# EI-CoreBioinformatics/portcullis

Measured on AMD Instinct MI355X. Metric: junc_reads_per_sec, higher is better.
Workload: dtype int32; 1 GPU; BASELINE configs[2]: synthetic 199999998 paired-end 150-bp reads, 25 contigs of GRCh38 lengths (3088286401 bp), 249999 junctions, orientation FR; reads_total=199999998, junctions_total=249999, contigs=25, reads_rank0=199999998, pairs_rank0=66692850

## Files before the change

### portcullis_amd/csrc/pjb_chain.hip.h

```cpp
#pragma once

constexpr unsigned K6_BLOCKS = 128;

static size_t rows_upper_bound(const pjb_ctx *c) {
    size_t n = c->rows_n;
    for (int k = 0; k < c->n_fl; k++)
        if (c->fl[k].queued) n += c->fl[k].lim.junc_limit;
    return n;
}

static void wait_flight(pjb_ctx *c, Flight &f) {
    if (f.queued) (void)hipEventSynchronize(c->sl[f.slot].ev_done);
}

static int rows_table_reserve(pjb_ctx *c, Flight &f, u32 JL) {
    size_t old = rows_upper_bound(c);
    if (old + JL <= c->rows_cap) return PJB_OK;
    for (int k = 0; k < c->n_fl; k++)
        if (c->fl[k].queued && &c->fl[k] != &f) wait_flight(c, c->fl[k]);
    int rc = rows_sync(c);
    if (rc) return rc;
    old = std::min(old, c->rows_cap);
    const size_t ncap = std::max<size_t>((old + JL) * 3 / 2, 1024);
    pjb_junction_row *nd = nullptr;
// ... 473 lines not shown
            else rc = sort_pass<u64>(ch, p == 0 ? S.okey.p : S.key[cur].p, S.key[cur ^ 1].p, vin, vout, shift, bits, ch.d_P, ch.rs_tiles, rs_names);
        }
        if (rc) return rc;
        cur ^= 1;
        shift += bits;
    }
    f.n_pass = ch.n_pass;
    if (ch.run_route) {
        const u32 *order = ch.ro_idx[cur];
        if ((rc = run_scan(c, ro_names[4], RunCountFn{(const u32 *)ro.cnt, order}, RunDestSink{ch.run_dest, order}, (u64)ch.run_cap, ch.ro_total, (const u32 *)ro.n_runs)))
            return rc;
        cur = 1;
        LAUNCH(c, ro_names[5], rs_place, dim3(ch.rs_tiles), dim3(256), (const u32 *)S.jidbam.p, ch.d_P, (const u64 *)ro.key, (const u32 *)ch.run_dest,
               (const u32 *)ro.tile_first, (const u32 *)ro.tile_n, ch.run_cap, ro.tile_bits, (u32 *)S.key[cur].p, (u32 *)S.idx[cur].p);
        f.n_pass = 1;
    }
    ch.cur = cur;
    f.sidx = (const u32 *)S.idx[cur].p;
    f.jid_sorted = f.lim.dense ? (const u32 *)S.key[cur].p : (const u32 *)S.jid.p;
    STAGE_EVENT(2);
    return PJB_OK;
}

static int chain_entropy(Chain &ch) {
    pjb_ctx *c = ch.c;
    CtlSlot &S = ch.S;
    LAUNCH(c, "k5_entropy_sum", k5_entropy_sum, dim3(std::max<u32>(1, (ch.JL + 15) / 16)), dim3(256), (const u32 *)S.seg.p, (const u32 *)S.runfirst.p,
           (const u32 *)S.runstart.p, ch.d_J, (double *)S.entsum.p);
    return PJB_OK;
}

#ifdef PJB_DEBUG_LAUNCH
static void debug_sort_check(Chain &ch) {
    Flight &f = ch.f;
    CtlSlot &S = ch.S;
    const int cur = ch.cur;
    fprintf(stderr, "[k4_pairs] tid %d PL %u JL %u slots_lim %u n_slices_lim %u frag cap %zu fragj cap %zu masks cap %zu rec cap %zu idx cap %zu key cap %zu jkey cap %zu cur %d n_pass %d\n",
            f.tid, ch.PL, ch.JL, ch.slots_lim, ch.n_slices_lim, S.frag.cap, S.fragj.cap, S.masks.cap, S.rec.cap, S.idx[cur].cap, S.key[cur].cap, S.jkey.cap, cur, f.n_pass);
    ContigStats hcs;
    (void)hipDeviceSynchronize();
    (void)hipMemcpy(&hcs, ch.d_cs, sizeof hcs, hipMemcpyDeviceToHost);
    u64 htot = 0;
    (void)hipMemcpy(&htot, S.total.p, 8, hipMemcpyDeviceToHost);
    fprintf(stderr, "[k4_pairs] cs: P %u n_pairs %llu J %u n_junc %u n_slots %u n_slices %u n_cand %u overflow %u R %u total %llu slot %d attempt %d\n", hcs.P,
            (unsigned long long)hcs.n_pairs, hcs.J, hcs.n_junc, hcs.n_slots, hcs.n_slices, hcs.n_cand, hcs.overflow, hcs.R, (unsigned long long)htot, f.slot, f.attempt);
    std::vector<u32> hs(hcs.P), hj(hcs.P), hb(hcs.P);
    (void)hipMemcpy(hs.data(), f.sidx, (size_t)hcs.P * 4, hipMemcpyDeviceToHost);
    (void)hipMemcpy(hj.data(), f.jid_sorted, (size_t)hcs.P * 4, hipMemcpyDeviceToHost);
    (void)hipMemcpy(hb.data(), S.jidbam.p, (size_t)hcs.P * 4, hipMemcpyDeviceToHost);
    std::vector<char> seen(hcs.P, 0);
    size_t bad_idx = 0, dup = 0, bad_order = 0, bad_in = 0, mism = 0;
    long first_bad = -1;
    for (size_t i = 0; i < hcs.P; i++) {
        if (hb[i] >= hcs.J) bad_in++;
        if (hs[i] >= hcs.P) {
            bad_idx++;
            if (first_bad < 0) first_bad = (long)i;
            continue;
        }
        if (seen[hs[i]]) dup++;
        seen[hs[i]] = 1;
        if (hj[i] != hb[hs[i]]) mism++;
        if (i && hj[i] < hj[i - 1]) bad_order++;
    }
    fprintf(stderr, "[k4_pairs] sort check: %zu indices out of range (first at %ld), %zu duplicates, %zu order breaks, %zu key/index mismatches, %zu input ids >= J\n", bad_idx,
            first_bad, dup, bad_order, mism, bad_in);
}
#endif

static int chain_runs_dense(Chain &ch) {
    pjb_ctx *c = ch.c;
    Flight &f = ch.f;
    CtlSlot &S = ch.S;
    const u32 n_slices_lim = ch.n_slices_lim, pair_blocks = ch.pair_blocks;
    int rc;
    u64 *head_mask = (u64 *)S.masks.p, *run_mask = head_mask + n_slices_lim;
    u32 *run_base = (u32 *)(run_mask + n_slices_lim);
    STAGE_EVENT(3);
    STAGE_EVENT(4);
    if (f.forked) HIP_TRY(c, hipStreamWaitEvent(ch.st, S.ev_join, 0));
#ifdef PJB_DEBUG_LAUNCH
    debug_sort_check(ch);
#endif
    LAUNCH(c, "k4_pairs", k4_pairs, dim3(pair_blocks), dim3(256), f.sidx, f.jid_sorted, (const PairRec *)ch.pr.rec, (const u64 *)S.jkey.p, ch.kf, ch.d_P,
           (u32 *)S.frag.p, (int32_t *)S.fragj.p, head_mask, run_mask, (const ContigStats *)ch.d_cs, ch.d_err);
    if ((rc = run_scan(c, "k2_runs", Popc64Fn{(const u64 *)run_mask}, ExclusiveU32Sink{run_base}, (u64)n_slices_lim, (u64 *)S.total.p, &ch.d_cs->n_slices)))
        return rc;
    LAUNCH(c, "k2_expand", k2_expand, dim3((pair_blocks + K2E_PER - 1) / K2E_PER), dim3(256), f.jid_sorted, (const u64 *)head_mask, (const u64 *)run_mask, (const u32 *)run_base,
           (const u64 *)S.total.p, (u32 *)S.seg.p, (u32 *)S.runfirst.p, (u32 *)S.runstart.p, ch.d_cs);
    STAGE_EVENT(5);
    return chain_fork(ch, S.ev_fork2, S.ev_join2, ch.entropy_forked, chain_entropy);
}

static int chain_runs_keys(Chain &ch) {
    pjb_ctx *c = ch.c;
    Flight &f = ch.f;
    CtlSlot &S = ch.S;
    const u32 JL = ch.JL, pair_blocks = ch.pair_blocks;
    int rc;
    const u64 *skey = (const u64 *)S.key[ch.cur].p;
    HeadFn hf{skey, f.sidx, (const PairRec *)ch.pr.rec};
    HeadSink hs{(u32 *)S.jid.p, (u32 *)S.seg.p, (u32 *)S.runfirst.p, (u32 *)S.runstart.p, skey, (u64 *)S.jkey.p, JL};
    if ((rc = run_scan(c, "k2_heads", hf, hs, (u64)ch.PL, (u64 *)S.total.p, ch.d_P))) return rc;
    LAUNCH(c, "k2_close", k2_close, dim3(1), dim3(1), (u64 *)S.total.p, (u32 *)S.seg.p, (u32 *)S.runfirst.p,
           (u32 *)S.runstart.p, ch.d_cs, JL, (const u32 *)ch.d_gen_cnt, ch.gen_cap);
    STAGE_EVENT(3);
    if ((rc = chain_fork(ch, S.ev_fork2, S.ev_join2, ch.entropy_forked, chain_entropy))) return rc;
    LAUNCH(c, "kf_init", kf_init, dim3(std::max<u32>(1, std::min<u32>((JL * F_WORDS + 255) / 256, 4096))), dim3(256), (u32 *)S.acc.p, ch.d_J, (int32_t *)S.ancl.p,
           (int32_t *)S.ancr.p);
    LAUNCH(c, "kf_anchors", kf_anchors, dim3(pair_blocks), dim3(256), f.sidx, (const u32 *)S.jid.p, (const PairRec *)ch.pr.rec, ch.d_P, (u32 *)S.jidbam.p,
           (int32_t *)S.ancl.p, (int32_t *)S.ancr.p);
    if ((rc = chain_k4b(ch))) return rc;
    STAGE_EVENT(4);
    LAUNCH(c, "k4_pairs", k4_pairs, dim3(pair_blocks), dim3(256), f.sidx, f.jid_sorted, (const PairRec *)ch.pr.rec, (const u64 *)S.jkey.p, ch.kf, ch.d_P,
           (u32 *)S.frag.p, (int32_t *)S.fragj.p, (u64 *)nullptr, (u64 *)nullptr, (const ContigStats *)ch.d_cs, ch.d_err);
    STAGE_EVENT(5);
    return PJB_OK;
}

static int chain_rows(Chain &ch) {
    pjb_ctx *c = ch.c;
    Flight &f = ch.f;
    CtlSlot &S = ch.S;
    const hipStream_t st = ch.st;
    const u32 JL = ch.JL;
    LAUNCH(c, "k5_frag_reduce", k5_frag_reduce, dim3((ch.slots_lim + 4 * FRAG_SLOTS_PER_WAVE - 1) / (4 * FRAG_SLOTS_PER_WAVE)), dim3(256),
           (const u32 *)S.frag.p, (const int32_t *)S.fragj.p, ch.d_slots, (u32 *)S.acc.p);
    if (ch.entropy_forked) HIP_TRY(c, hipStreamWaitEvent(st, S.ev_join2, 0));
    LAUNCH(c, "k5_finalize", k5_finalize, dim3(std::max<u32>(1, (JL + 255) / 256)), dim3(256), (const u64 *)S.jkey.p, (const u32 *)S.seg.p,
           (const u32 *)S.runfirst.p, (const u32 *)S.runstart.p, (const u32 *)S.acc.p,
           (const int32_t *)S.ancl.p, (const int32_t *)S.ancr.p, ch.kf, ch.GT, ch.d_J, (const double *)S.entsum.p, (pjb_junction_row *)S.rows.p, ch.d_err,
           ch.d_member_junc);
    STAGE_EVENT(6);
    u64 *mirror_table = nullptr;
    u32 mirror_room = 0;
    if (c->mirror && c->mirror_cap >= PJB_MIRROR_HEADER_BYTES) {
        mirror_table = (u64 *)(c->mirror + PJB_MIRROR_HEADER_BYTES);
        mirror_room = (u32)std::min<size_t>((c->mirror_cap - PJB_MIRROR_HEADER_BYTES) / sizeof(pjb_junction_row), 0xffffffffu);
    }
    const hipStream_t rows_stream = c->side_stream ? c->stream3 : st;
    if (rows_stream != st) {
        HIP_TRY(c, hipEventRecord(S.ev_rows, st));
        HIP_TRY(c, hipStreamWaitEvent(rows_stream, S.ev_rows, 0));
    }
    {
        ChainScope scope{c};
        c->stream = rows_stream;
        LAUNCH(c, "k6_rows_out", k6_rows_out, dim3(K6_BLOCKS), dim3(256), (const u64 *)S.rows.p, (const ContigStats *)ch.d_cs,
               (u64 *)c->rows_table, ch.row_base, ch.mirror_base, (RowCursor *)c->b_cursor.p, mirror_table, mirror_room, ch.d_err, ch.d_gen_cnt, S.pub_dev,
               (const MemberStats *)ch.d_members, ch.d_member_junc, ch.n_members);
    }
    S.at_rest = true;
    HIP_TRY(c, hipEventRecord(S.ev[7], rows_stream));
    HIP_TRY(c, hipEventRecord(S.ev_done, rows_stream));
    f.queued = true;
    return PJB_OK;
}
#undef STAGE_EVENT

static int queue_contig(pjb_ctx *c, Flight &f) {
    Chain ch{c, f, c->sl[f.slot]};
    int rc = chain_plan(ch);
    ChainScope scope{c};
    c->stream = ch.st;
    c->scan_tiles = &ch.S.scan_tiles;
    c->cur_pool = c->cur_slot = f.slot;
    ev_drop(c, f.slot);
    if (rc || (rc = chain_room(ch)) || (rc = chain_front(ch)) || (rc = chain_k1(ch)) || (rc = chain_k2d(ch)) || (rc = chain_sort(ch)) ||
        (rc = f.lim.dense ? chain_runs_dense(ch) : chain_runs_keys(ch)))
        return rc;
    return chain_rows(ch);
}
```

### portcullis_amd/csrc/pjb_kernels.hip.h

```cpp
#pragma once

#include "pjb_device.hip.h"

namespace pjb {

__global__ __launch_bounds__(256) void k0_upper(uint8_t *g, int64_t n, int do_upper, int *has_x) {
    int64_t i = ((int64_t)blockIdx.x * 256 + threadIdx.x) * 16;
    bool x = false;
    for (int64_t j = i; j < n && j < i + 16; j++) {
        uint8_t c = g[j];
        x |= (c == 'X' || (do_upper && c == 'x'));
    }
    if (__ballot(x) && lane_id() == 0) atomicOr(has_x, 1);
    if (!do_upper) return;
    if (i + 16 <= n && ((uintptr_t)(g + i) & 15) == 0) {
        uint4 v = *reinterpret_cast<uint4 *>(g + i);
        u32 *w = reinterpret_cast<u32 *>(&v);
#pragma unroll
        for (int k = 0; k < 4; k++) {
            u32 x = w[k], r = 0;
#pragma unroll
            for (int b = 0; b < 4; b++) {
                u32 c = (x >> (8 * b)) & 0xff;
                if (c >= 'a' && c <= 'z') c -= 32;
// ... 1929 lines not shown
        const u32 q = base + threadIdx.x;
        const bool on = q < n;
        const u32 pc = on ? q : n - 1;
        const u32 rs = cand_rank[pc];
        const u64 k = cand[pc], a = cand_anc[pc];
        bool valid = on && rs < junc_limit;
        u32 id = 0xffffffffu;
        if (valid) {
            int32_t s, e;
            unpack_key(kf, k, s, e);
            id = first_id[rs] + ends_below(ends, rs, (u32)e);
            valid = id < junc_limit;
            if (valid) jkey[id] = k;
        }
        if (valid) {
            const int32_t lo = (int32_t)(u32)a, hi = (int32_t)(u32)(a >> 32);
            if (lo < __hip_atomic_load(&anc_l[id], __ATOMIC_RELAXED, __HIP_MEMORY_SCOPE_AGENT)) atomicMin(&anc_l[id], lo);
            if (hi > __hip_atomic_load(&anc_r[id], __ATOMIC_RELAXED, __HIP_MEMORY_SCOPE_AGENT)) atomicMax(&anc_r[id], hi);
        }
    }
}

enum {
    F_N = 0, F_R1P, F_R1N, F_R2P, F_R2N, F_MS, F_XSP, F_XSN, F_UM, F_BPP, F_PPP, F_REL, F_DIST,
    F_MAXMINANC, F_UP, F_DOWN, F_MAXMMES, F_MAXMINMATCH,
    F_FIRSTMIS,
    F_PAD19,
    F_MISM_LO, F_MISM_HI,
    F_JAD0,
    F_WORDS = 48
};
__device__ __forceinline__ void acc_rest_state(u32 *acc, u64 n_junc) {
    const u64 n = n_junc * F_WORDS, step = (u64)gridDim.x * blockDim.x;
    for (u64 t = (u64)blockIdx.x * blockDim.x + threadIdx.x; t < n; t += step) acc[t] = (t % F_WORDS) == F_FIRSTMIS ? 100000000u : 0u;
}

constexpr int KDA_TILE = 4096;
__device__ __forceinline__ void wave_hist_add(u32 *h, u32 d, bool valid);
constexpr int KDA_PER = 4;
constexpr u32 RUN_W = 2048;
struct RunOut {
    u64 *key;
    u32 *cnt;
    u32 *tile_first;
    u32 *tile_n;
    u32 *n_runs;
    u32 cap;
    u32 window;
    int tile_bits;
};
static_assert(RUN_W == 256 * 8, "kd_assign compacts eight table entries a thread");
__device__ __forceinline__ void runs_close_chain(ContigStats *cs) {
    atomicOr(&cs->overflow, OVF_RUNS);
    cs->P = 0;
    cs->J = 0;
    cs->n_slots = 0;
    cs->n_slices = 0;
}
__global__ __launch_bounds__(256) void kd_assign(const u64 *key, const u32 *np, KeyFmt kf, const u64 *bitmap, const u32 *wrank, const u32 *ends,
                                                 const u32 *first_id, u32 junc_limit, const u64 *total, u32 *jid_bam, u32 *acc, const u64 *jkey,
                                                 const int32_t *anc_l, const int32_t *anc_r, u64 *err, ContigStats *cs_chk, int hist_bits, u32 *hist,
                                                 RunOut ro) {
    __shared__ u32 s_h[4096];
    __shared__ u32 s_run[4];
    __shared__ u32 s_rscan[4];
    const u32 n = *np;
    if (n == 0) {
        if (hist_bits > 0)
            for (u32 d = threadIdx.x; d < (1u << hist_bits); d += 256) hist[(size_t)blockIdx.x * (1u << hist_bits) + d] = 0;
        return;
    }
    {
        const u64 J = *total;
        acc_rest_state(acc, J < (u64)junc_limit ? J : (u64)junc_limit);
    }
    const u32 nb = hist_bits > 0 ? 1u << hist_bits : 0u;
    for (u32 d = threadIdx.x; d < (ro.window ? RUN_W : nb); d += 256) s_h[d] = 0;
    if (threadIdx.x == 0) {
        s_run[0] = 0xffffffffu;
        s_run[1] = 0u;
    }
    if (nb || ro.window) __syncthreads();
    u32 id_lo = 0xffffffffu, id_hi = 0u;
    for (u32 chunk = blockIdx.x * (KDA_TILE / (KDA_PER * 256)); chunk < (blockIdx.x + 1) * (KDA_TILE / (KDA_PER * 256)); chunk++) {
    if (chunk * (KDA_PER * 256) >= n) break;
    u64 kk[KDA_PER];
    u32 pp[KDA_PER];
#pragma unroll
    for (int q = 0; q < KDA_PER; q++) {
        pp[q] = (chunk * KDA_PER + q) * 256 + threadIdx.x;
        kk[q] = key[pp[q] < n ? pp[q] : n - 1];
    }
    bool lead[KDA_PER];
    int32_t ss[KDA_PER], ee[KDA_PER];
    u64 bw[KDA_PER];
    u32 wr[KDA_PER];
#pragma unroll
    for (int q = 0; q < KDA_PER; q++) {
        const u32 plo = (u32)__builtin_amdgcn_update_dpp(0, (int)(u32)kk[q], 0x138, 0xf, 0xf, false);
        const u32 phi = (u32)__builtin_amdgcn_update_dpp(0, (int)(u32)(kk[q] >> 32), 0x138, 0xf, 0xf, false);
        lead[q] = lane_id() == 0 || plo != (u32)kk[q] || phi != (u32)(kk[q] >> 32);
        unpack_key(kf, kk[q], ss[q], ee[q]);
        bw[q] = 0;
        wr[q] = 0;
        if (lead[q]) {
            bw[q] = bitmap[(u32)ss[q] >> 6];
            wr[q] = wrank[(u32)ss[q] >> 6];
        }
    }
    u32 rs_[KDA_PER], fi[KDA_PER], eb[KDA_PER];
#pragma unroll
    for (int q = 0; q < KDA_PER; q++) {
        rs_[q] = wr[q] + (u32)__popcll(bw[q] & ((1ull << (ss[q] & 63)) - 1ull));
        fi[q] = eb[q] = 0;
        if (lead[q]) {
            fi[q] = first_id[rs_[q]];
            eb[q] = ends_below(ends, rs_[q], (u32)ee[q]);
        }
    }
#pragma unroll
    for (int q = 0; q < KDA_PER; q++) {
        const u64 lm = __ballot(lead[q]) & ((2ull << lane_id()) - 1ull);
        const u32 id = (u32)__shfl((int)(fi[q] + eb[q]), 63 - __clzll((long long)lm), 64);
        fi[q] = id;
        eb[q] = 0;
        if (pp[q] < n) jid_bam[pp[q]] = id;
        if (nb) wave_hist_add(s_h, id & (nb - 1u), pp[q] < n);
        if (ro.window) {
            wave_hist_add(s_h, id & (RUN_W - 1u), pp[q] < n);
            if (pp[q] < n) {
                id_lo = id < id_lo ? id : id_lo;
                id_hi = id > id_hi ? id : id_hi;
            }
        }
    }
#ifdef PJB_SELFCHECK
    const u32 p = pp[0];
    if (p < n) {
    const int32_t s = ss[0], e = ee[0];
    const u32 rs = rs_[0], id = fi[0] + eb[0];
    {
        int bad = 0;
        const uint4 *q = reinterpret_cast<const uint4 *>(ends + (size_t)rs * DENSE_ENDS);
        const uint4 a = q[0], b = q[1];
        const u32 ue = (u32)e;
        if (!((bitmap[(u32)s >> 6] >> (s & 63)) & 1ull)) bad = 6;
        else if (!(a.x == ue || a.y == ue || a.z == ue || a.w == ue || b.x == ue || b.y == ue || b.z == ue || b.w == ue)) bad = 7;
        else if (id >= junc_limit || id >= (u32)*total) bad = 1;
        else if (jkey[id] != key[p]) bad = 2;
        else if (anc_l[id] > s || anc_r[id] < e) bad = 3;
        if (bad) {
            set_error(err, 0xfffff000u + (u32)bad, PJB_ERR_HIP);
            cs_chk->P = 0;
        }
    }
    }
#endif
    }
    if (nb) {
        __syncthreads();
        for (u32 d = threadIdx.x; d < nb; d += 256) hist[(size_t)blockIdx.x * nb + d] = s_h[d];
    }
    if (ro.window) {
        id_lo = wave_total<DppMin>(id_lo);
        id_hi = wave_total<DppMax>(id_hi);
        if (lane_id() == 0) {
            atomicMin(&s_run[0], id_lo);
            atomicMax(&s_run[1], id_hi);
        }
        __syncthreads();
        const u32 lo = s_run[0], hi = s_run[1];
        if (lo > hi) {
            if (threadIdx.x == 0) ro.tile_n[blockIdx.x] = 0;
            return;
        }
        if (hi - lo >= ro.window) {
            if (threadIdx.x == 0) {
                ro.tile_n[blockIdx.x] = 0;
                runs_close_chain(cs_chk);
            }
            return;
        }
        const u32 span = hi - lo + 1u;
        u32 c[8], nz = 0;
#pragma unroll
        for (int k = 0; k < 8; k++) {
            const u32 o = threadIdx.x * 8u + (u32)k;
            c[k] = o < span ? s_h[(lo + o) & (RUN_W - 1u)] : 0u;
            nz += c[k] != 0u;
        }
        u32 tot;
        u32 at = block_escan_256<u32>(nz, s_rscan, &tot);
        if (threadIdx.x == 0) {
            u32 b = atomicAdd(ro.n_runs, tot);
            if (b > ro.cap || tot > ro.cap - b) {
                atomicSub(ro.n_runs, tot);
                b = 0xffffffffu;
                runs_close_chain(cs_chk);
            }
            s_run[2] = b;
            ro.tile_first[blockIdx.x] = b == 0xffffffffu ? 0u : b;
            ro.tile_n[blockIdx.x] = b == 0xffffffffu ? 0u : tot;
        }
        __syncthreads();
        const u32 first = s_run[2];
        if (first == 0xffffffffu) return;
        at += first;
#pragma unroll
        for (int k = 0; k < 8; k++)
            if (c[k]) {
                ro.key[at] = ((u64)(lo + threadIdx.x * 8u + (u32)k) << ro.tile_bits) | (u64)blockIdx.x;
                ro.cnt[at] = c[k];
                at++;
            }
    }
}

constexpr int RS_ITEMS = 16;
constexpr int RS_TILE = 256 * RS_ITEMS;
constexpr int RS_MAX_BITS = 12;
constexpr int RS_MAX_BINS = 1 << RS_MAX_BITS;
static_assert(KDA_TILE == RS_TILE && RS_MAX_BINS <= 4096, "kd_assign counts the sort's first digit tile by tile");

__device__ __forceinline__ void wave_hist_add(u32 *h, u32 d, bool valid) {
    u64 rem = __ballot(valid);
    const int lane = lane_id();
#pragma unroll
    for (int it = 0; it < 2; it++) {
        if (rem == 0) return;
        const int first = __ffsll((long long)rem) - 1;
        const u32 d0 = __shfl(d, first, 64);
        const u64 m = __ballot(valid && d == d0) & rem;
        if (lane == first) atomicAdd(&h[d0], (u32)__popcll(m));
        rem &= ~m;
    }
    if ((rem >> lane) & 1ull) atomicAdd(&h[d], 1u);
}

template <typename K>
__global__ __launch_bounds__(256) void rs_hist(const K *keys, const u32 *np, int shift, int bits, u32 *hist, u32 n_tiles) {
// ... 608 lines not shown
        if (threadIdx.x == 255) s_first[2 * GEN_SHARDS] = total;
        __syncthreads();
    }
    static_assert(GEN_SHARDS == 256, "two sub-lists per thread of the block");
    const u32 n_items = s_first[2 * GEN_SHARDS];
    for (u32 item0 = blockIdx.x * 256; item0 < n_items; item0 += gridDim.x * 256) {
    const u32 item = item0 + threadIdx.x;
    if (item >= n_items) continue;
    u32 sub = 0;
#pragma unroll
    for (u32 step = GEN_SHARDS; step > 0; step >>= 1)
        if (sub + step < 2 * GEN_SHARDS && s_first[sub + step] <= item) sub += step;
    const bool check_only = sub >= GEN_SHARDS;
    const u64 entry = list[(size_t)sub * cap + (item - s_first[sub])];
    const u32 p0 = (u32)(entry >> 32);
    const u32 slot = check_only && pack_nn ? (u32)entry & 0x0fffffffu : (u32)entry;
    if (check_only) {
        const u32 code = pack_nn ? (u32)entry >> 28 : 15u;
        const u32 nN = code < 15u ? code : (reinterpret_cast<const uint4 *>(rec + p0)[1].w >> 16) + 1u;
        bool ok = true;
        int32_t prev_istart = 0, is, ie;
        unpack_key(kf, key[p0], is, ie);
        for (u32 k = 0; k < nN; k++) {
            const u32 j = jid_bam[p0 + k];
            int32_t nis = 0, nie = 0;
            if (k + 1 < nN) unpack_key(kf, key[p0 + k + 1], nis, nie);
            if (k > 0 && prev_istart >= anc_l[j]) ok = false;
            if (k + 1 < nN && nie + 1 <= anc_r[j]) ok = false;
            prev_istart = is;
            is = nis;
            ie = nie;
        }
        if (ok) continue;
    }
    const int bi = s_bt.find(batches, n_batches, slot / (u32)K1_TILE);
    const DevBatch &b = batches[bi];
    const u32 r = spl_idx[slot];
    const uint4 sr = spl_rec[slot];
    const u32 g = gload(&b.base) + r;
    const u32 c0 = sr.x;
    u32 nc = sr.w & 0x7fffu;
    if (nc == 0x7fffu) nc = gload(b.cig_off + r + 1) - c0;
    OpsView cig;
    cig.g = b.cigar + c0;
    cig.lds = &s_ops[0][threadIdx.x];
    {
        u32 w[OPS_LDS];
        fetch_ops8(as_global(b.cigar), c0, s_bt.cig_words(b, bi), w);
#pragma unroll
        for (int k = 0; k < OPS_LDS; k++) s_ops[k][threadIdx.x] = (u32)k < nc ? w[k] : 0u;
    }
    const uint4 rb = reinterpret_cast<const uint4 *>(rec + p0)[1];
    const int32_t vpos = (int32_t)rb.x, aend = (int32_t)rb.y;
    const Member M = member_of(G, vpos);
    const int32_t pos = vpos - M.voff;
    int32_t lq = (int32_t)(sr.w >> 16);
    if (lq == 0xffff) lq = gload(b.l_qseq + r);
    const u32 so0 = sr.z;
    if (lq > 1 && !(sr.w & 0x8000u)) {
        set_error(err, g, PJB_ERR_NO_SEQ);
        continue;
    }
    const uint8_t *seq = b.seq4 + (size_t)so0 * 4;
    const int32_t q_limit = (int32_t)min(s_bt.seq_words(b, bi) - 1u - so0, 0x7fffffffu);
    u32 k = 0;
    int32_t qsum = 0;
    for (u32 i = 0; i < nc; i++) {
        const u32 op = cig[i], ty = op & 15u;
        if (ty == OP_N) {
            const u32 p = p0 + k;
            const u32 j = jid_bam[p];
            int32_t istart, iend;
            unpack_key(kf, key[p], istart, iend);
            const u64 res = pair_stats_generic(cig, nc, pos, aend - vpos + 1, seq, lq, M.d, M.len, genome_has_x != 0, use_codes ? M.codes : (const u32 *)nullptr,
                                               anc_l[j] - M.voff, istart - M.voff, iend - M.voff, anc_r[j] - M.voff, g, err, i, qsum, q_limit);
            *reinterpret_cast<u64 *>(rec + p) = res;
            k++;
        }
        if (op_consumes_query(ty) && ty != OP_S) qsum += (int32_t)(op >> 4);
    }
    }
}

__global__ __launch_bounds__(256) void k4_pairs(const u32 *sidx, const u32 *jid_of, const PairRec *rec, const u64 *jkey, KeyFmt kf, const u32 *np,
                                                 u32 *frag, int32_t *frag_j, u64 *head_mask, u64 *run_mask, const ContigStats *cs_chk, u64 *err_chk) {
    const u32 n = *np;
    if (blockIdx.x * 256u >= n) return;
    const u32 i = blockIdx.x * 256 + threadIdx.x;
    const bool valid = i < n;
    const int lane = lane_id();
    const u32 ic = valid ? i : n - 1;
    const u32 p = sidx[ic];
    const u32 jv = jid_of[ic];
#ifdef PJB_SELFCHECK
    {
        const u32 Jc = cs_chk->J;
        const u32 jb = ic ? jid_of[ic - 1] : jv;
        int bad = 0;
        if (p >= n) bad = 1;
        else if (jv >= Jc) bad = 2;
        else if (jv != jb && jv != jb + 1) bad = 3;
        else if (ic == 0 && jv != 0) bad = 4;
        else if (ic == n - 1 && jv != Jc - 1) bad = 5;
        else if (jv + (ic >> 6) + 1 >= cs_chk->n_slots) bad = 6;
        else if ((ic >> 6) >= cs_chk->n_slices) bad = 7;
        else if (cs_chk->n_slots != Jc + (n + 63) / 64) bad = 8;
        if (__ballot(bad != 0)) {
            if (bad) set_error(err_chk, 0xffffe000u + (u32)bad, PJB_ERR_HIP);
            return;
        }
    }
#endif
    const PairRec Rc = rec_load(rec + p);
    const u64 jk = jkey[jv];
    u32 jprev_v = __shfl_up(jv, 1, 64);
    int32_t pos_prev = __shfl_up(Rc.pos, 1, 64), aend_prev = __shfl_up(Rc.aend, 1, 64);
    if (lane == 0 && valid && i > 0) {
        jprev_v = jid_of[i - 1];
        const uint4 q = reinterpret_cast<const uint4 *>(rec + sidx[i - 1])[1];
        pos_prev = (int32_t)q.x;
        aend_prev = (int32_t)q.y;
    }
    u32 j = 0xffffffffu;
    u32 cnt[4] = {0, 0, 0, 0}, jadp[5] = {0, 0, 0, 0, 0}, mx[5] = {0, 0, 0, 0, 0};
    u32 first_mis = 100000000u;
    u64 mism64 = 0;
    if (valid) {
        j = jv;
        int32_t istart, iend;
        unpack_key(kf, jk, istart, iend);
        const u64 rs = Rc.aux;
        const u32 minMatch = (u32)(rs & 0xfffffu), mmes = (u32)((rs >> 20) & 0xfffffu), nbMis = (u32)(rs >> 40);
        const u32 meta = Rc.meta;
        const u32 cat = meta & META_CAT_MASK;
        const u32 xs = (meta >> META_XS_SHIFT) & 3u;
        const bool dist_head = i == 0 || jprev_v != j || pos_prev != Rc.pos || aend_prev != Rc.aend;
        cnt[0] = 1u | ((u32)(cat == 0) << 8) | ((u32)(cat == 1) << 16) | ((u32)(cat == 2) << 24);
        cnt[1] = (u32)(cat == 3) | ((u32)((meta & META_MULTI) != 0) << 8) | ((u32)(xs == 1) << 16) | ((u32)(xs == 2) << 24);
        cnt[2] = (u32)((meta & META_UM) != 0) | ((u32)((meta & META_BPP) != 0) << 8) | ((u32)((meta & META_PPP) != 0) << 16) |
                 ((u32)((meta & META_REL) != 0) << 24);
        cnt[3] = (u32)dist_head;
#pragma unroll
        for (int w = 0; w < 5; w++)
            jadp[w] = (u32)((u32)(4 * w) < minMatch) | ((u32)((u32)(4 * w + 1) < minMatch) << 8) |
                      ((u32)((u32)(4 * w + 2) < minMatch) << 16) | ((u32)((u32)(4 * w + 3) < minMatch) << 24);
        const int32_t la = istart - Rc.lstart, ra = Rc.rend - iend;
        mx[0] = (u32)(la < ra ? la : ra);
        mx[1] = Rc.updown & 0xffffu;
        mx[2] = Rc.updown >> 16;
        mx[3] = mmes;
        mx[4] = minMatch;
        first_mis = minMatch > 0 ? minMatch : 100000000u;
        mism64 = nbMis;
        if (lane == 0 && i > 0 && jprev_v != j) frag_j[j + (i >> 6) - 1] = -1;
        if (i == n - 1) frag_j[j + (i >> 6) + 1] = -1;
    }
    if (head_mask) {
        const bool hj = valid && (i == 0 || jprev_v != j);
        const bool hr = valid && (hj || pos_prev != Rc.pos);
        const u64 mj = __ballot(hj), mr = __ballot(hr);
        if (lane == 0 && i < n) {
            head_mask[i >> 6] = mj;
            run_mask[i >> 6] = mr;
        }
    }
    auto store_fragment = [&](u32 hi_word) {
        const u32 slot = j + (i >> 6);
        u32 vals[F_WORDS];
#pragma unroll
        for (int k = 0; k < F_WORDS; k++) vals[k] = 0;
#pragma unroll
        for (int k = 0; k < 13; k++) vals[F_N + k] = (cnt[k >> 2] >> (8 * (k & 3))) & 0xffu;
        vals[F_MAXMINANC] = mx[0];
        vals[F_UP] = mx[1];
        vals[F_DOWN] = mx[2];
        vals[F_MAXMMES] = mx[3];
        vals[F_MAXMINMATCH] = mx[4];
        vals[F_FIRSTMIS] = first_mis;
        vals[F_MISM_LO] = (u32)mism64;
        vals[F_MISM_HI] = hi_word;
#pragma unroll
        for (int k = 0; k < 20; k++) vals[F_JAD0 + k] = (jadp[k >> 2] >> (8 * (k & 3))) & 0xffu;
        uint4 *dst = reinterpret_cast<uint4 *>(frag + (size_t)slot * F_WORDS);
#pragma unroll
        for (int k = 0; k < F_WORDS / 4; k++) dst[k] = make_uint4(vals[4 * k], vals[4 * k + 1], vals[4 * k + 2], vals[4 * k + 3]);
        frag_j[slot] = (int32_t)j;
    };
    const u32 j0 = (u32)__builtin_amdgcn_readfirstlane((int)j);
    if (__ballot(valid && j != j0) == 0) {
#pragma unroll
        for (int w = 0; w < 4; w++) cnt[w] = wave_total<DppAdd>(cnt[w]);
#pragma unroll
        for (int w = 0; w < 5; w++) jadp[w] = wave_total<DppAdd>(jadp[w]);
#pragma unroll
        for (int w = 0; w < 5; w++) mx[w] = wave_total<DppMax>(mx[w]);
        first_mis = wave_total<DppMin>(first_mis);
        mism64 = (u64)wave_total<DppAdd>((u32)mism64);
        if (valid && lane == 0) store_fragment(0u);
        return;
    }
    u32 take = 0;
#pragma unroll
    for (int sft = 0; sft < 6; sft++) {
        const int o = 1 << sft;
        const u32 kk = __shfl_down(j, o, 64);
        if (lane + o < 64 && kk == j) take |= 1u << sft;
    }
    auto red_add = [&](u32 v) {
#pragma unroll
        for (int sft = 0; sft < 6; sft++) {
            const u32 t = __shfl_down(v, 1 << sft, 64);
            if ((take >> sft) & 1u) v += t;
        }
        return v;
    };
    auto red_max = [&](u32 v) {
#pragma unroll
        for (int sft = 0; sft < 6; sft++) {
            const u32 t = __shfl_down(v, 1 << sft, 64);
            if (((take >> sft) & 1u) && t > v) v = t;
        }
        return v;
    };
#pragma unroll
    for (int w = 0; w < 4; w++) cnt[w] = red_add(cnt[w]);
#pragma unroll
    for (int w = 0; w < 5; w++) jadp[w] = red_add(jadp[w]);
#pragma unroll
    for (int w = 0; w < 5; w++) mx[w] = red_max(mx[w]);
#pragma unroll
    for (int sft = 0; sft < 6; sft++) {
        const u32 t = __shfl_down(first_mis, 1 << sft, 64);
        const u64 t64 = __shfl_down(mism64, 1 << sft, 64);
        if ((take >> sft) & 1u) {
            first_mis = t < first_mis ? t : first_mis;
            mism64 += t64;
        }
    }
    const u32 jprev = __shfl_up(j, 1, 64);
    if (valid && (lane == 0 || jprev != j)) store_fragment((u32)(mism64 >> 32));
}

__device__ __forceinline__ u32 frag_combine(int k, u32 a, u32 b) {
    if (k >= F_MAXMINANC && k <= F_MAXMINMATCH) return a > b ? a : b;
    if (k == F_FIRSTMIS) return a < b ? a : b;
    return a + b;
}
constexpr int FRAG_SLOTS_PER_WAVE = 16;
__global__ __launch_bounds__(256) void k5_frag_reduce(const u32 *frag, const int32_t *frag_j, const u32 *n_slots_p, u32 *acc) {
    const u32 n_slots = *n_slots_p;
    const u32 wave = (blockIdx.x * 256 + threadIdx.x) >> 6;
    const int k = lane_id();
    const u32 s0 = wave * FRAG_SLOTS_PER_WAVE;
    if (s0 >= n_slots) return;
    const int32_t myj = (k < FRAG_SLOTS_PER_WAVE && s0 + k < n_slots) ? frag_j[s0 + k] : -1;
    int32_t cur = -1;
    u32 v = 0, carry_lo = 0;
    auto flush = [&](int32_t j) {
        if (j < 0 || k >= F_JAD0 + 20) return;
        u32 *dst = acc + (size_t)j * F_WORDS + k;
        if (k == F_MISM_LO) return;
        if (k == F_MISM_HI) {
            atomicAdd(reinterpret_cast<u64 *>(dst - 1), ((u64)v << 32) | carry_lo);
        } else if (k >= F_MAXMINANC && k <= F_MAXMINMATCH) atomicMax(dst, v);
        else if (k == F_FIRSTMIS) atomicMin(dst, v);
        else if (v) atomicAdd(dst, v);
    };
    u32 row[FRAG_SLOTS_PER_WAVE];
#pragma unroll
    for (int q = 0; q < FRAG_SLOTS_PER_WAVE; q++) {
        const int32_t jq = __shfl(myj, q, 64);
        row[q] = (jq >= 0 && k < F_WORDS) ? frag[(size_t)(s0 + (u32)q) * F_WORDS + k] : 0u;
    }
#pragma unroll
    for (int q = 0; q < FRAG_SLOTS_PER_WAVE; q++) {
        const int32_t j = __shfl(myj, q, 64);
        if (j >= 0) {
            const u32 w = row[q];
            const u32 wlo = __shfl(w, F_MISM_LO, 64);
            if (j != cur) {
                flush(cur);
                cur = j;
                v = w;
                carry_lo = wlo;
            } else if (k == F_MISM_HI) {
                const u64 sum = (((u64)v << 32) | carry_lo) + (((u64)w << 32) | wlo);
                v = (u32)(sum >> 32);
                carry_lo = (u32)sum;
            } else {
                v = frag_combine(k, v, w);
            }
        }
    }
    flush(cur);
}


__global__ __launch_bounds__(256) void k5_entropy_sum(const u32 *seg_off, const u32 *run_first, const u32 *run_start, const u32 *n_junc_p,
                                                       double *ent_sum) {
    const int lane = lane_id(), sl = lane & 15;
    const u32 j = ((blockIdx.x * 4 + (threadIdx.x >> 6)) << 2) + (u32)(lane >> 4);
    const bool valid = j < *n_junc_p;
    const u32 rf = valid ? run_first[j] : 0u, rl = valid ? run_first[j + 1] : 0u;
    const u32 n = valid ? seg_off[j + 1] - seg_off[j] : 0u;
    double sum = 0.0;
    for (u32 r0 = rf; __any(r0 < rl); r0 += 16) {
        const u32 r = r0 + (u32)sl;
        double t = 0.0;
        if (r < rl) {
            u32 c = run_start[r + 1] - run_start[r];
            if (rl - rf > 1) {
                if (r == rf) c += 1;
                else if (r == rl - 1) c -= 1;
            }
            if (c != 0 && n > 1) {
                const double pI = (double)c / (double)n;
                t = __dmul_rn(pI, log2(pI));
            }
        }
        const u32 cnt = r0 < rl ? (rl - r0 < 16u ? rl - r0 : 16u) : 0u;
#pragma unroll
        for (u32 k = 0; k < 16; k++) {
            const double v = __shfl(t, (int)k, 16);
// ... 238 lines not shown
```

Baseline: 30.03 billion reads/s.

## Process multiple slices per wave in k4_pairs and software-pipeline dense-assign chunks

k4_pairs now handles K4_PER consecutive 64-element slices per wave. When all of them share one junction, it folds their counters into a single fragment using widened 16-bit lanes and marks the other fragment slots empty with -1. Previous-element context for later slices comes from readlane instead of a global reload, and the launch grid shrinks to match. Separately, the dense-assign kernel's chunk loop is restructured into staged lambdas so that key loads and bitmap lookups for later chunks are issued before the current chunk finishes, hiding memory latency at the cost of more registers.

```diff
diff --git a/portcullis_amd/csrc/pjb_chain.hip.h b/portcullis_amd/csrc/pjb_chain.hip.h
--- a/portcullis_amd/csrc/pjb_chain.hip.h
+++ b/portcullis_amd/csrc/pjb_chain.hip.h
@@ -579,7 +579,7 @@
 #ifdef PJB_DEBUG_LAUNCH
     debug_sort_check(ch);
 #endif
-    LAUNCH(c, "k4_pairs", k4_pairs, dim3(pair_blocks), dim3(256), f.sidx, f.jid_sorted, (const PairRec *)ch.pr.rec, (const u64 *)S.jkey.p, ch.kf, ch.d_P,
+    LAUNCH(c, "k4_pairs", k4_pairs, dim3((pair_blocks + K4_PER - 1) / K4_PER), dim3(256), f.sidx, f.jid_sorted, (const PairRec *)ch.pr.rec, (const u64 *)S.jkey.p, ch.kf, ch.d_P,
            (u32 *)S.frag.p, (int32_t *)S.fragj.p, head_mask, run_mask, (const ContigStats *)ch.d_cs, ch.d_err);
     if ((rc = run_scan(c, "k2_runs", Popc64Fn{(const u64 *)run_mask}, ExclusiveU32Sink{run_base}, (u64)n_slices_lim, (u64 *)S.total.p, &ch.d_cs->n_slices)))
         return rc;
@@ -609,7 +609,7 @@
            (int32_t *)S.ancl.p, (int32_t *)S.ancr.p);
     if ((rc = chain_k4b(ch))) return rc;
     STAGE_EVENT(4);
-    LAUNCH(c, "k4_pairs", k4_pairs, dim3(pair_blocks), dim3(256), f.sidx, f.jid_sorted, (const PairRec *)ch.pr.rec, (const u64 *)S.jkey.p, ch.kf, ch.d_P,
+    LAUNCH(c, "k4_pairs", k4_pairs, dim3((pair_blocks + K4_PER - 1) / K4_PER), dim3(256), f.sidx, f.jid_sorted, (const PairRec *)ch.pr.rec, (const u64 *)S.jkey.p, ch.kf, ch.d_P,
            (u32 *)S.frag.p, (int32_t *)S.fragj.p, (u64 *)nullptr, (u64 *)nullptr, (const ContigStats *)ch.d_cs, ch.d_err);
     STAGE_EVENT(5);
     return PJB_OK;
diff --git a/portcullis_amd/csrc/pjb_kernels.hip.h b/portcullis_amd/csrc/pjb_kernels.hip.h
--- a/portcullis_amd/csrc/pjb_kernels.hip.h
+++ b/portcullis_amd/csrc/pjb_kernels.hip.h
@@ -2035,80 +2035,103 @@
     }
     if (nb || ro.window) __syncthreads();
     u32 id_lo = 0xffffffffu, id_hi = 0u;
-    for (u32 chunk = blockIdx.x * (KDA_TILE / (KDA_PER * 256)); chunk < (blockIdx.x + 1) * (KDA_TILE / (KDA_PER * 256)); chunk++) {
-    if (chunk * (KDA_PER * 256) >= n) break;
-    u64 kk[KDA_PER];
-    u32 pp[KDA_PER];
-#pragma unroll
-    for (int q = 0; q < KDA_PER; q++) {
-        pp[q] = (chunk * KDA_PER + q) * 256 + threadIdx.x;
-        kk[q] = key[pp[q] < n ? pp[q] : n - 1];
-    }
-    bool lead[KDA_PER];
-    int32_t ss[KDA_PER], ee[KDA_PER];
-    u64 bw[KDA_PER];
-    u32 wr[KDA_PER];
-#pragma unroll
-    for (int q = 0; q < KDA_PER; q++) {
-        const u32 plo = (u32)__builtin_amdgcn_update_dpp(0, (int)(u32)kk[q], 0x138, 0xf, 0xf, false);
-        const u32 phi = (u32)__builtin_amdgcn_update_dpp(0, (int)(u32)(kk[q] >> 32), 0x138, 0xf, 0xf, false);
-        lead[q] = lane_id() == 0 || plo != (u32)kk[q] || phi != (u32)(kk[q] >> 32);
-        unpack_key(kf, kk[q], ss[q], ee[q]);
-        bw[q] = 0;
-        wr[q] = 0;
-        if (lead[q]) {
-            bw[q] = bitmap[(u32)ss[q] >> 6];
-            wr[q] = wrank[(u32)ss[q] >> 6];
-        }
-    }
-    u32 rs_[KDA_PER], fi[KDA_PER], eb[KDA_PER];
-#pragma unroll
-    for (int q = 0; q < KDA_PER; q++) {
-        rs_[q] = wr[q] + (u32)__popcll(bw[q] & ((1ull << (ss[q] & 63)) - 1ull));
-        fi[q] = eb[q] = 0;
-        if (lead[q]) {
-            fi[q] = first_id[rs_[q]];
-            eb[q] = ends_below(ends, rs_[q], (u32)ee[q]);
-        }
-    }
-#pragma unroll
-    for (int q = 0; q < KDA_PER; q++) {
-        const u64 lm = __ballot(lead[q]) & ((2ull << lane_id()) - 1ull);
-        const u32 id = (u32)__shfl((int)(fi[q] + eb[q]), 63 - __clzll((long long)lm), 64);
-        fi[q] = id;
-        eb[q] = 0;
-        if (pp[q] < n) jid_bam[pp[q]] = id;
-        if (nb) wave_hist_add(s_h, id & (nb - 1u), pp[q] < n);
-        if (ro.window) {
-            wave_hist_add(s_h, id & (RUN_W - 1u), pp[q] < n);
-            if (pp[q] < n) {
-                id_lo = id < id_lo ? id : id_lo;
-                id_hi = id > id_hi ? id : id_hi;
-            }
-        }
-    }
+    constexpr int KDA_CHUNKS = KDA_TILE / (KDA_PER * 256);
+    u64 kk[KDA_CHUNKS][KDA_PER];
+    u32 pp[KDA_CHUNKS][KDA_PER];
+    bool lead[KDA_CHUNKS][KDA_PER];
+    int32_t ss[KDA_CHUNKS][KDA_PER], ee[KDA_CHUNKS][KDA_PER];
+    u64 bw[KDA_CHUNKS][KDA_PER];
+    u32 wr[KDA_CHUNKS][KDA_PER];
+    u32 rs_[KDA_CHUNKS][KDA_PER], fi[KDA_CHUNKS][KDA_PER], eb[KDA_CHUNKS][KDA_PER];
+    const auto live = [&](int c) __attribute__((always_inline)) {
+        return c < KDA_CHUNKS && (u64)(blockIdx.x * (u32)KDA_CHUNKS + (u32)c) * (u64)(KDA_PER * 256) < (u64)n;
+    };
+    const auto ask_keys = [&](int c) __attribute__((always_inline)) {
+        if (!live(c)) return;
+#pragma unroll
+        for (int q = 0; q < KDA_PER; q++) {
+            pp[c][q] = ((blockIdx.x * (u32)KDA_CHUNKS + (u32)c) * KDA_PER + q) * 256 + threadIdx.x;
+            kk[c][q] = key[pp[c][q] < n ? pp[c][q] : n - 1];
+        }
+    };
+    const auto ask_words = [&](int c) __attribute__((always_inline)) {
+        if (!live(c)) return;
+#pragma unroll
+        for (int q = 0; q < KDA_PER; q++) {
+            const u32 plo = (u32)__builtin_amdgcn_update_dpp(0, (int)(u32)kk[c][q], 0x138, 0xf, 0xf, false);
+            const u32 phi = (u32)__builtin_amdgcn_update_dpp(0, (int)(u32)(kk[c][q] >> 32), 0x138, 0xf, 0xf, false);
+            lead[c][q] = lane_id() == 0 || plo != (u32)kk[c][q] || phi != (u32)(kk[c][q] >> 32);
+            unpack_key(kf, kk[c][q], ss[c][q], ee[c][q]);
+            bw[c][q] = 0;
+            wr[c][q] = 0;
+            if (lead[c][q]) {
+                bw[c][q] = bitmap[(u32)ss[c][q] >> 6];
+                wr[c][q] = wrank[(u32)ss[c][q] >> 6];
+            }
+        }
+    };
+    const auto ask_slots = [&](int c) __attribute__((always_inline)) {
+        if (!live(c)) return;
+#pragma unroll
+        for (int q = 0; q < KDA_PER; q++) {
+            rs_[c][q] = wr[c][q] + (u32)__popcll(bw[c][q] & ((1ull << (ss[c][q] & 63)) - 1ull));
+            fi[c][q] = eb[c][q] = 0;
+            if (lead[c][q]) {
+                fi[c][q] = first_id[rs_[c][q]];
+                eb[c][q] = ends_below(ends, rs_[c][q], (u32)ee[c][q]);
+            }
+        }
+    };
+    const auto finish = [&](int c) __attribute__((always_inline)) {
+        if (!live(c)) return;
+#pragma unroll
+        for (int q = 0; q < KDA_PER; q++) {
+            const u64 lm = __ballot(lead[c][q]) & ((2ull << lane_id()) - 1ull);
+            const u32 id = (u32)__shfl((int)(fi[c][q] + eb[c][q]), 63 - __clzll((long long)lm), 64);
+            fi[c][q] = id;
+            eb[c][q] = 0;
+            if (pp[c][q] < n) jid_bam[pp[c][q]] = id;
+            if (nb) wave_hist_add(s_h, id & (nb - 1u), pp[c][q] < n);
+            if (ro.window) {
+                wave_hist_add(s_h, id & (RUN_W - 1u), pp[c][q] < n);
+                if (pp[c][q] < n) {
+                    id_lo = id < id_lo ? id : id_lo;
+                    id_hi = id > id_hi ? id : id_hi;
+                }
+            }
+        }
 #ifdef PJB_SELFCHECK
-    const u32 p = pp[0];
-    if (p < n) {
-    const int32_t s = ss[0], e = ee[0];
-    const u32 rs = rs_[0], id = fi[0] + eb[0];
-    {
-        int bad = 0;
-        const uint4 *q = reinterpret_cast<const uint4 *>(ends + (size_t)rs * DENSE_ENDS);
-        const uint4 a = q[0], b = q[1];
-        const u32 ue = (u32)e;
-        if (!((bitmap[(u32)s >> 6] >> (s & 63)) & 1ull)) bad = 6;
-        else if (!(a.x == ue || a.y == ue || a.z == ue || a.w == ue || b.x == ue || b.y == ue || b.z == ue || b.w == ue)) bad = 7;
-        else if (id >= junc_limit || id >= (u32)*total) bad = 1;
-        else if (jkey[id] != key[p]) bad = 2;
-        else if (anc_l[id] > s || anc_r[id] < e) bad = 3;
-        if (bad) {
-            set_error(err, 0xfffff000u + (u32)bad, PJB_ERR_HIP);
-            cs_chk->P = 0;
-        }
-    }
-    }
+        const u32 p = pp[c][0];
+        if (p < n) {
+        const int32_t s = ss[c][0], e = ee[c][0];
+        const u32 rs = rs_[c][0], id = fi[c][0] + eb[c][0];
+        {
+            int bad = 0;
+            const uint4 *q = reinterpret_cast<const uint4 *>(ends + (size_t)rs * DENSE_ENDS);
+            const uint4 a = q[0], b = q[1];
+            const u32 ue = (u32)e;
+            if (!((bitmap[(u32)s >> 6] >> (s & 63)) & 1ull)) bad = 6;
+            else if (!(a.x == ue || a.y == ue || a.z == ue || a.w == ue || b.x == ue || b.y == ue || b.z == ue || b.w == ue)) bad = 7;
+            else if (id >= junc_limit || id >= (u32)*total) bad = 1;
+            else if (jkey[id] != key[p]) bad = 2;
+            else if (anc_l[id] > s || anc_r[id] < e) bad = 3;
+            if (bad) {
+                set_error(err, 0xfffff000u + (u32)bad, PJB_ERR_HIP);
+                cs_chk->P = 0;
+            }
+        }
+        }
 #endif
+    };
+    ask_keys(0);
+    ask_words(0);
+    ask_keys(1);
+#pragma unroll
+    for (int c = 0; c < KDA_CHUNKS; c++) {
+        ask_slots(c);
+        ask_words(c + 1);
+        ask_keys(c + 2);
+        finish(c);
     }
     if (nb) {
         __syncthreads();
@@ -2883,59 +2906,131 @@
     }
 }
 
+constexpr int K4_PER = 2;
+static_assert(K4_PER >= 1 && K4_PER * 64 < 65536 && K4_PER < 256, "the folded sums travel in 16-bit lanes, a lane's own in 8-bit lanes");
 __global__ __launch_bounds__(256) void k4_pairs(const u32 *sidx, const u32 *jid_of, const PairRec *rec, const u64 *jkey, KeyFmt kf, const u32 *np,
                                                  u32 *frag, int32_t *frag_j, u64 *head_mask, u64 *run_mask, const ContigStats *cs_chk, u64 *err_chk) {
     const u32 n = *np;
-    if (blockIdx.x * 256u >= n) return;
-    const u32 i = blockIdx.x * 256 + threadIdx.x;
-    const bool valid = i < n;
     const int lane = lane_id();
-    const u32 ic = valid ? i : n - 1;
-    const u32 p = sidx[ic];
-    const u32 jv = jid_of[ic];
+    const u32 slice0 = (u32)__builtin_amdgcn_readfirstlane((int)((blockIdx.x * 4u + (threadIdx.x >> 6)) * (u32)K4_PER));
+    if ((u64)slice0 * 64u >= n) return;
+    u32 ii[K4_PER], pp[K4_PER], jv[K4_PER];
+#pragma unroll
+    for (int s = 0; s < K4_PER; s++) {
+        ii[s] = (slice0 + (u32)s) * 64u + (u32)lane;
+        const u32 ic = ii[s] < n ? ii[s] : n - 1;
+        pp[s] = sidx[ic];
+        jv[s] = jid_of[ic];
+    }
+    const bool fetch_before = slice0 > 0;
+    u32 p_before = 0, j_before = 0;
+    if (fetch_before) {
+        p_before = sidx[slice0 * 64u - 1u];
+        j_before = jid_of[slice0 * 64u - 1u];
+    }
 #ifdef PJB_SELFCHECK
     {
         const u32 Jc = cs_chk->J;
-        const u32 jb = ic ? jid_of[ic - 1] : jv;
         int bad = 0;
-        if (p >= n) bad = 1;
-        else if (jv >= Jc) bad = 2;
-        else if (jv != jb && jv != jb + 1) bad = 3;
-        else if (ic == 0 && jv != 0) bad = 4;
-        else if (ic == n - 1 && jv != Jc - 1) bad = 5;
-        else if (jv + (ic >> 6) + 1 >= cs_chk->n_slots) bad = 6;
-        else if ((ic >> 6) >= cs_chk->n_slices) bad = 7;
-        else if (cs_chk->n_slots != Jc + (n + 63) / 64) bad = 8;
+#pragma unroll
+        for (int s = 0; s < K4_PER; s++) {
+            const u32 ic = ii[s] < n ? ii[s] : n - 1;
+            const u32 p = pp[s], jvs = jv[s];
+            const u32 jb = ic ? jid_of[ic - 1] : jvs;
+            if (bad) continue;
+            if (p >= n) bad = 1;
+            else if (jvs >= Jc) bad = 2;
+            else if (jvs != jb && jvs != jb + 1) bad = 3;
+            else if (ic == 0 && jvs != 0) bad = 4;
+            else if (ic == n - 1 && jvs != Jc - 1) bad = 5;
+            else if (jvs + (ic >> 6) + 1 >= cs_chk->n_slots) bad = 6;
+            else if ((ic >> 6) >= cs_chk->n_slices) bad = 7;
+            else if (cs_chk->n_slots != Jc + (n + 63) / 64) bad = 8;
+        }
         if (__ballot(bad != 0)) {
             if (bad) set_error(err_chk, 0xffffe000u + (u32)bad, PJB_ERR_HIP);
             return;
         }
     }
 #endif
-    const PairRec Rc = rec_load(rec + p);
-    const u64 jk = jkey[jv];
-    u32 jprev_v = __shfl_up(jv, 1, 64);
-    int32_t pos_prev = __shfl_up(Rc.pos, 1, 64), aend_prev = __shfl_up(Rc.aend, 1, 64);
-    if (lane == 0 && valid && i > 0) {
-        jprev_v = jid_of[i - 1];
-        const uint4 q = reinterpret_cast<const uint4 *>(rec + sidx[i - 1])[1];
-        pos_prev = (int32_t)q.x;
-        aend_prev = (int32_t)q.y;
+    PairRec Rc[K4_PER];
+    u64 jk[K4_PER];
+#pragma unroll
+    for (int s = 0; s < K4_PER; s++) {
+        Rc[s] = rec_load(rec + pp[s]);
+        jk[s] = jkey[jv[s]];
+    }
+    int32_t pos_before = 0, aend_before = 0;
+    if (fetch_before) {
+        const uint4 q = reinterpret_cast<const uint4 *>(rec + p_before)[1];
+        pos_before = (int32_t)q.x;
+        aend_before = (int32_t)q.y;
+    }
+    auto store_fragment = [&](u32 slot, u32 jj, auto sum_of, auto jad_of, const u32(&mxv)[5], u32 fm, u32 mis_lo, u32 mis_hi) {
+        u32 vals[F_WORDS];
+#pragma unroll
+        for (int k = 0; k < F_WORDS; k++) vals[k] = 0;
+#pragma unroll
+        for (int k = 0; k < 13; k++) vals[F_N + k] = sum_of(k);
+        vals[F_MAXMINANC] = mxv[0];
+        vals[F_UP] = mxv[1];
+        vals[F_DOWN] = mxv[2];
+        vals[F_MAXMMES] = mxv[3];
+        vals[F_MAXMINMATCH] = mxv[4];
+        vals[F_FIRSTMIS] = fm;
+        vals[F_MISM_LO] = mis_lo;
+        vals[F_MISM_HI] = mis_hi;
+#pragma unroll
+        for (int k = 0; k < 20; k++) vals[F_JAD0 + k] = jad_of(k);
+        uint4 *dst = reinterpret_cast<uint4 *>(frag + (size_t)slot * F_WORDS);
+#pragma unroll
+        for (int k = 0; k < F_WORDS / 4; k++) dst[k] = make_uint4(vals[4 * k], vals[4 * k + 1], vals[4 * k + 2], vals[4 * k + 3]);
+        frag_j[slot] = (int32_t)jj;
+    };
+    const u32 jw = (u32)__builtin_amdgcn_readfirstlane((int)jv[0]);
+    bool other = false;
+#pragma unroll
+    for (int s = 0; s < K4_PER; s++) other = other || (ii[s] < n && jv[s] != jw);
+    const bool fold = __ballot(other) == 0;
+    u32 fcnt[4] = {0, 0, 0, 0}, fjad[5] = {0, 0, 0, 0, 0}, fmx[5] = {0, 0, 0, 0, 0};
+    u32 ffirst = 100000000u, fmis = 0;
+#pragma unroll
+    for (int s = 0; s < K4_PER; s++) {
+    if ((u64)(slice0 + (u32)s) * 64u < n) {
+    const u32 i = ii[s];
+    const bool valid = i < n;
+    const PairRec &R = Rc[s];
+    u32 jprev_v = __shfl_up(jv[s], 1, 64);
+    int32_t pos_prev = __shfl_up(R.pos, 1, 64), aend_prev = __shfl_up(R.aend, 1, 64);
+    if (s == 0) {
+        if (fetch_before && lane == 0) {
+            jprev_v = j_before;
+            pos_prev = pos_before;
+            aend_prev = aend_before;
+        }
+    } else {
+        const u32 jl = (u32)__builtin_amdgcn_readlane((int)jv[s > 0 ? s - 1 : 0], 63);
+        const int32_t pl = __builtin_amdgcn_readlane(Rc[s > 0 ? s - 1 : 0].pos, 63), al = __builtin_amdgcn_readlane(Rc[s > 0 ? s - 1 : 0].aend, 63);
+        if (lane == 0) {
+            jprev_v = jl;
+            pos_prev = pl;
+            aend_prev = al;
+        }
     }
     u32 j = 0xffffffffu;
     u32 cnt[4] = {0, 0, 0, 0}, jadp[5] = {0, 0, 0, 0, 0}, mx[5] = {0, 0, 0, 0, 0};
     u32 first_mis = 100000000u;
     u64 mism64 = 0;
     if (valid) {
-        j = jv;
+        j = jv[s];
         int32_t istart, iend;
-        unpack_key(kf, jk, istart, iend);
-        const u64 rs = Rc.aux;
+        unpack_key(kf, jk[s], istart, iend);
+        const u64 rs = R.aux;
         const u32 minMatch = (u32)(rs & 0xfffffu), mmes = (u32)((rs >> 20) & 0xfffffu), nbMis = (u32)(rs >> 40);
-        const u32 meta = Rc.meta;
+        const u32 meta = R.meta;
         const u32 cat = meta & META_CAT_MASK;
         const u32 xs = (meta >> META_XS_SHIFT) & 3u;
-        const bool dist_head = i == 0 || jprev_v != j || pos_prev != Rc.pos || aend_prev != Rc.aend;
+        const bool dist_head = i == 0 || jprev_v != j || pos_prev != R.pos || aend_prev != R.aend;
         cnt[0] = 1u | ((u32)(cat == 0) << 8) | ((u32)(cat == 1) << 16) | ((u32)(cat == 2) << 24);
         cnt[1] = (u32)(cat == 3) | ((u32)((meta & META_MULTI) != 0) << 8) | ((u32)(xs == 1) << 16) | ((u32)(xs == 2) << 24);
         cnt[2] = (u32)((meta & META_UM) != 0) | ((u32)((meta & META_BPP) != 0) << 8) | ((u32)((meta & META_PPP) != 0) << 16) |
@@ -2945,10 +3040,10 @@
         for (int w = 0; w < 5; w++)
             jadp[w] = (u32)((u32)(4 * w) < minMatch) | ((u32)((u32)(4 * w + 1) < minMatch) << 8) |
                       ((u32)((u32)(4 * w + 2) < minMatch) << 16) | ((u32)((u32)(4 * w + 3) < minMatch) << 24);
-        const int32_t la = istart - Rc.lstart, ra = Rc.rend - iend;
+        const int32_t la = istart - R.lstart, ra = R.rend - iend;
         mx[0] = (u32)(la < ra ? la : ra);
-        mx[1] = Rc.updown & 0xffffu;
-        mx[2] = Rc.updown >> 16;
+        mx[1] = R.updown & 0xffffu;
+        mx[2] = R.updown >> 16;
         mx[3] = mmes;
         mx[4] = minMatch;
         first_mis = minMatch > 0 ? minMatch : 100000000u;
@@ -2958,37 +3053,27 @@
     }
     if (head_mask) {
         const bool hj = valid && (i == 0 || jprev_v != j);
-        const bool hr = valid && (hj || pos_prev != Rc.pos);
+        const bool hr = valid && (hj || pos_prev != R.pos);
         const u64 mj = __ballot(hj), mr = __ballot(hr);
-        if (lane == 0 && i < n) {
+        if (lane == 0) {
             head_mask[i >> 6] = mj;
             run_mask[i >> 6] = mr;
         }
     }
-    auto store_fragment = [&](u32 hi_word) {
-        const u32 slot = j + (i >> 6);
-        u32 vals[F_WORDS];
-#pragma unroll
-        for (int k = 0; k < F_WORDS; k++) vals[k] = 0;
-#pragma unroll
-        for (int k = 0; k < 13; k++) vals[F_N + k] = (cnt[k >> 2] >> (8 * (k & 3))) & 0xffu;
-        vals[F_MAXMINANC] = mx[0];
-        vals[F_UP] = mx[1];
-        vals[F_DOWN] = mx[2];
-        vals[F_MAXMMES] = mx[3];
-        vals[F_MAXMINMATCH] = mx[4];
-        vals[F_FIRSTMIS] = first_mis;
-        vals[F_MISM_LO] = (u32)mism64;
-        vals[F_MISM_HI] = hi_word;
-#pragma unroll
-        for (int k = 0; k < 20; k++) vals[F_JAD0 + k] = (jadp[k >> 2] >> (8 * (k & 3))) & 0xffu;
-        uint4 *dst = reinterpret_cast<uint4 *>(frag + (size_t)slot * F_WORDS);
-#pragma unroll
-        for (int k = 0; k < F_WORDS / 4; k++) dst[k] = make_uint4(vals[4 * k], vals[4 * k + 1], vals[4 * k + 2], vals[4 * k + 3]);
-        frag_j[slot] = (int32_t)j;
-    };
-    const u32 j0 = (u32)__builtin_amdgcn_readfirstlane((int)j);
-    if (__ballot(valid && j != j0) == 0) {
+    const auto sum8 = [&](int k) { return (cnt[k >> 2] >> (8 * (k & 3))) & 0xffu; };
+    const auto jad8 = [&](int k) { return (jadp[k >> 2] >> (8 * (k & 3))) & 0xffu; };
+    const u32 js = (u32)__builtin_amdgcn_readfirstlane((int)j);
+    if (fold) {
+#pragma unroll
+        for (int w = 0; w < 4; w++) fcnt[w] += cnt[w];
+#pragma unroll
+        for (int w = 0; w < 5; w++) fjad[w] += jadp[w];
+#pragma unroll
+        for (int w = 0; w < 5; w++) fmx[w] = mx[w] > fmx[w] ? mx[w] : fmx[w];
+        ffirst = first_mis < ffirst ? first_mis : ffirst;
+        fmis += (u32)mism64;
+        if (s > 0 && lane == 0) frag_j[jw + slice0 + (u32)s] = -1;
+    } else if (__ballot(valid && j != js) == 0) {
 #pragma unroll
         for (int w = 0; w < 4; w++) cnt[w] = wave_total<DppAdd>(cnt[w]);
 #pragma unroll
@@ -2997,49 +3082,71 @@
         for (int w = 0; w < 5; w++) mx[w] = wave_total<DppMax>(mx[w]);
         first_mis = wave_total<DppMin>(first_mis);
         mism64 = (u64)wave_total<DppAdd>((u32)mism64);
-        if (valid && lane == 0) store_fragment(0u);
-        return;
-    }
-    u32 take = 0;
-#pragma unroll
-    for (int sft = 0; sft < 6; sft++) {
-        const int o = 1 << sft;
-        const u32 kk = __shfl_down(j, o, 64);
-        if (lane + o < 64 && kk == j) take |= 1u << sft;
-    }
-    auto red_add = [&](u32 v) {
+        if (lane == 0) store_fragment(j + (i >> 6), j, sum8, jad8, mx, first_mis, (u32)mism64, 0u);
+    } else {
+        u32 take = 0;
 #pragma unroll
         for (int sft = 0; sft < 6; sft++) {
-            const u32 t = __shfl_down(v, 1 << sft, 64);
-            if ((take >> sft) & 1u) v += t;
-        }
-        return v;
-    };
-    auto red_max = [&](u32 v) {
+            const int o = 1 << sft;
+            const u32 kk = __shfl_down(j, o, 64);
+            if (lane + o < 64 && kk == j) take |= 1u << sft;
+        }
+        auto red_add = [&](u32 v) {
+#pragma unroll
+            for (int sft = 0; sft < 6; sft++) {
+                const u32 t = __shfl_down(v, 1 << sft, 64);
+                if ((take >> sft) & 1u) v += t;
+            }
+            return v;
+        };
+        auto red_max = [&](u32 v) {
+#pragma unroll
+            for (int sft = 0; sft < 6; sft++) {
+                const u32 t = __shfl_down(v, 1 << sft, 64);
+                if (((take >> sft) & 1u) && t > v) v = t;
+            }
+            return v;
+        };
+#pragma unroll
+        for (int w = 0; w < 4; w++) cnt[w] = red_add(cnt[w]);
+#pragma unroll
+        for (int w = 0; w < 5; w++) jadp[w] = red_add(jadp[w]);
+#pragma unroll
+        for (int w = 0; w < 5; w++) mx[w] = red_max(mx[w]);
 #pragma unroll
         for (int sft = 0; sft < 6; sft++) {
-            const u32 t = __shfl_down(v, 1 << sft, 64);
-            if (((take >> sft) & 1u) && t > v) v = t;
-        }
-        return v;
-    };
-#pragma unroll
-    for (int w = 0; w < 4; w++) cnt[w] = red_add(cnt[w]);
-#pragma unroll
-    for (int w = 0; w < 5; w++) jadp[w] = red_add(jadp[w]);
-#pragma unroll
-    for (int w = 0; w < 5; w++) mx[w] = red_max(mx[w]);
-#pragma unroll
-    for (int sft = 0; sft < 6; sft++) {
-        const u32 t = __shfl_down(first_mis, 1 << sft, 64);
-        const u64 t64 = __shfl_down(mism64, 1 << sft, 64);
-        if ((take >> sft) & 1u) {
-            first_mis = t < first_mis ? t : first_mis;
-            mism64 += t64;
-        }
-    }
-    const u32 jprev = __shfl_up(j, 1, 64);
-    if (valid && (lane == 0 || jprev != j)) store_fragment((u32)(mism64 >> 32));
+            const u32 t = __shfl_down(first_mis, 1 << sft, 64);
+            const u64 t64 = __shfl_down(mism64, 1 << sft, 64);
+            if ((take >> sft) & 1u) {
+                first_mis = t < first_mis ? t : first_mis;
+                mism64 += t64;
+            }
+        }
+        const u32 jprev = __shfl_up(j, 1, 64);
+        if (valid && (lane == 0 || jprev != j)) store_fragment(j + (i >> 6), j, sum8, jad8, mx, first_mis, (u32)mism64, (u32)(mism64 >> 32));
+    }
+    }
+    }
+    if (fold) {
+        u32 lo[4], hi[3], jlo[5], jhi[5];
+#pragma unroll
+        for (int w = 0; w < 4; w++) lo[w] = wave_total<DppAdd>(fcnt[w] & 0x00ff00ffu);
+#pragma unroll
+        for (int w = 0; w < 3; w++) hi[w] = wave_total<DppAdd>((fcnt[w] >> 8) & 0x00ff00ffu);
+#pragma unroll
+        for (int w = 0; w < 5; w++) {
+            jlo[w] = wave_total<DppAdd>(fjad[w] & 0x00ff00ffu);
+            jhi[w] = wave_total<DppAdd>((fjad[w] >> 8) & 0x00ff00ffu);
+        }
+#pragma unroll
+        for (int w = 0; w < 5; w++) fmx[w] = wave_total<DppMax>(fmx[w]);
+        ffirst = wave_total<DppMin>(ffirst);
+        static_assert(K4_PER * 64 <= 256, "the folded mismatch sum is a 32-bit word");
+        fmis = wave_total<DppAdd>(fmis);
+        const auto sum16 = [&](int k) { return (((k & 1) ? hi[(k >> 2) < 3 ? (k >> 2) : 0] : lo[k >> 2]) >> (16 * ((k >> 1) & 1))) & 0xffffu; };
+        const auto jad16 = [&](int k) { return (((k & 1) ? jhi[k >> 2] : jlo[k >> 2]) >> (16 * ((k >> 1) & 1))) & 0xffffu; };
+        if (lane == 0) store_fragment(jw + slice0, jw, sum16, jad16, fmx, ffirst, fmis, 0u);
+    }
 }
 
 __device__ __forceinline__ u32 frag_combine(int k, u32 a, u32 b) {
```

Measured after the change: 30.27 billion reads/s, median of 2. Within noise of the previous version (+0.8%).
